# cyberfabric/cyberfabric-core

Hardware: AMD Instinct MI355X
Metric: tokens/sec + p50 TTFT via llm-gateway REST /v1/chat/completions (higher is better)
Workload: dtype bf16; 1 GPU; model=llama3-8b, global_batch=2048, seq_len=512, parallelism=dp1(worker fleet)

## Files before the change

### csrc/attn_paged.hip

```cpp
#include <float.h>

#include "common.h"

#define ATTN_BS 16

template <int GROUP, int D>
__global__ __launch_bounds__(256) void paged_attn_kernel(
    bf16* __restrict__ out, const bf16* __restrict__ q,
    const bf16* __restrict__ k_cache, const bf16* __restrict__ v_cache,
    const int* __restrict__ block_tables, const int* __restrict__ ctx_lens,
    const int* __restrict__ row_seq, int max_blocks, int num_kv_heads,
    float scale, long q_stride) {
  constexpr int SLICE = D / 4;
  constexpr int VPL = D / 64;
  constexpr bool QREG = (GROUP <= 4);
  const int row = blockIdx.x;
  const int kvh = blockIdx.y;
  const int H = num_kv_heads * GROUP;
  const int ctx = ctx_lens[row];
  const int table = row_seq ? row_seq[row] : row;
  const int* bt = block_tables + (long)table * max_blocks;
  const int nblocks = (ctx + ATTN_BS - 1) / ATTN_BS;

  __shared__ __attribute__((aligned(16))) float q_lds[GROUP][D];
// ... 149 lines not shown
  }
  __syncthreads();
  for (int i = threadIdx.x; i < GROUP * D; i += 256) {
    const int h = i / D, d = i % D;
    float M = fmaxf(fmaxf(comb_m[0][h], comb_m[1][h]),
                    fmaxf(comb_m[2][h], comb_m[3][h]));
    float o = 0.f, L = 0.f;
    #pragma unroll
    for (int w = 0; w < 4; ++w) {
      const float f = (comb_m[w][h] == -FLT_MAX) ? 0.f
                                                 : __expf(comb_m[w][h] - M);
      o += f * comb_o[w][h][d];
      L += f * comb_l[w][h];
    }
    *(unsigned short*)(out + ((long)row * H + kvh * GROUP + h) * D + d) =
        f2bf(o / L);
  }
}


DEV float dot2_bf16(unsigned a, unsigned b, float c) {
  asm("v_dot2_f32_bf16 %0, %1, %2, %0" : "+v"(c) : "v"(a), "v"(b));
  return c;
}

typedef __attribute__((ext_vector_type(2))) float float2v;

DEV unsigned pk_bf16(float a, float b) {
  unsigned r;
  asm("v_cvt_pk_bf16_f32 %0, %1, %2" : "=v"(r) : "v"(a), "v"(b));
  return r;
}

template <int GROUP, bool KV8>
__global__ __launch_bounds__(256) void paged_attn_v3_kernel(
    bf16* __restrict__ out, const bf16* __restrict__ q,
    const bf16* __restrict__ k_cache, const bf16* __restrict__ v_cache,
    const int* __restrict__ block_tables, const int* __restrict__ ctx_lens,
    const int* __restrict__ row_seq, int max_blocks, int num_kv_heads,
    float scale, long q_stride, int h_total, int g_stride, int h_off,
    float* __restrict__ partial) {
  constexpr int D = 128;
  const int row = blockIdx.x;
  const int kvh = blockIdx.y;
  const int split = gridDim.z;
  const int H = h_total;
  const int ctx = ctx_lens[row];
  const int table = row_seq ? row_seq[row] : row;
  const int* bt = block_tables + (long)table * max_blocks;
  const int nblocks = (ctx + ATTN_BS - 1) / ATTN_BS;

  __shared__ __attribute__((aligned(16))) float sc[4][GROUP][ATTN_BS];
  __shared__ __attribute__((aligned(16))) float comb_o[4][GROUP][D];
  __shared__ float comb_m[4][GROUP];
  __shared__ float comb_l[4][GROUP];

  const int wid = threadIdx.x >> 6;
  const int lane = threadIdx.x & 63;
  const int t_loc = lane >> 3;
  const int sl = lane & 7;
  const int ds = lane & 15;
  const int g = lane >> 4;

  unsigned q_pk[GROUP][8];
  {
    const bf16* qp = q + (long)row * q_stride
                     + ((long)kvh * g_stride + h_off) * D + sl * 16;
    #pragma unroll
    for (int h = 0; h < GROUP; ++h) {
      uint4 a = *reinterpret_cast<const uint4*>(qp + h * D);
      uint4 b = *reinterpret_cast<const uint4*>(qp + h * D + 8);
      q_pk[h][0] = a.x; q_pk[h][1] = a.y; q_pk[h][2] = a.z; q_pk[h][3] = a.w;
      q_pk[h][4] = b.x; q_pk[h][5] = b.y; q_pk[h][6] = b.z; q_pk[h][7] = b.w;
    }
  }

  float m[GROUP], l[GROUP];
  float2 acc[GROUP][4];
  #pragma unroll
  for (int h = 0; h < GROUP; ++h) {
    m[h] = -FLT_MAX; l[h] = 0.f;
    #pragma unroll
    for (int j = 0; j < 4; ++j) acc[h][j] = make_float2(0.f, 0.f);
  }

  for (int b = 4 * blockIdx.z + wid; b < nblocks; b += 4 * split) {
    const long blk = bt[b];
    const int nb = min(ATTN_BS, ctx - b * ATTN_BS);
    const long page_off = ((blk * num_kv_heads + kvh) * ATTN_BS) * D;
    const bf16* pbase = k_cache + page_off;
    const bf16* vbase = v_cache + page_off;
    const unsigned char* pbase8 =
        reinterpret_cast<const unsigned char*>(k_cache) + page_off;
    const unsigned char* vbase8 =
        reinterpret_cast<const unsigned char*>(v_cache) + page_off;
    uint4 kr[2][KV8 ? 1 : 2];
    uint4 vr4[KV8 ? 1 : 4];
    uint2 vr2[KV8 ? 4 : 1];
    #pragma unroll
    for (int p = 0; p < 2; ++p) {
      if constexpr (KV8) {
        kr[p][0] = *reinterpret_cast<const uint4*>(
            pbase8 + (p * 8 + t_loc) * D + sl * 16);
      } else {
        const bf16* kp = pbase + (p * 8 + t_loc) * D + sl * 16;
        kr[p][0] = *reinterpret_cast<const uint4*>(kp);
        kr[p][1] = *reinterpret_cast<const uint4*>(kp + 8);
      }
    }
    #pragma unroll
    for (int i = 0; i < 4; ++i) {
      if constexpr (KV8)
        vr2[i] = *reinterpret_cast<const uint2*>(vbase8 + (4 * g + i) * D
                                                 + ds * 8);
      else
        vr4[i] = *reinterpret_cast<const uint4*>(vbase + (4 * g + i) * D
                                                 + ds * 8);
    }
    float s[GROUP][2];
    #pragma unroll
    for (int p = 0; p < 2; ++p) {
      unsigned kw[8];
      if constexpr (KV8) {
        const unsigned* kq = reinterpret_cast<const unsigned*>(&kr[p][0]);
        #pragma unroll
        for (int i = 0; i < 4; ++i) {
          float2v lo = __builtin_amdgcn_cvt_pk_f32_fp8(kq[i], false);
          float2v hi = __builtin_amdgcn_cvt_pk_f32_fp8(kq[i], true);
          kw[2 * i] = pk_bf16(lo.x, lo.y);
          kw[2 * i + 1] = pk_bf16(hi.x, hi.y);
        }
      } else {
        #pragma unroll
        for (int j = 0; j < 8; ++j)
          kw[j] = reinterpret_cast<const unsigned*>(&kr[p][0])[j];
      }
      #pragma unroll
      for (int h = 0; h < GROUP; ++h) {
        float d = 0.f;
        #pragma unroll
        for (int j = 0; j < 8; ++j) d = dot2_bf16(q_pk[h][j], kw[j], d);
        d += __shfl_xor(d, 1);
        d += __shfl_xor(d, 2);
        d += __shfl_xor(d, 4);
        const int tok = p * 8 + t_loc;
        s[h][p] = (tok < nb) ? d * scale : -FLT_MAX;
      }
    }
    #pragma unroll
    for (int h = 0; h < GROUP; ++h) {
      float bm = fmaxf(s[h][0], s[h][1]);
// ... 24 lines not shown
    #pragma unroll
    for (int h = 0; h < GROUP; ++h)
      p4[h] = *reinterpret_cast<const float4*>(&sc[wid][h][4 * g]);
    #pragma unroll
    for (int i = 0; i < 4; ++i) {
      float2 vf[4];
      if constexpr (KV8) {
        const unsigned* vw = reinterpret_cast<const unsigned*>(&vr2[i]);
        #pragma unroll
        for (int jj = 0; jj < 2; ++jj) {
          float2v lo = __builtin_amdgcn_cvt_pk_f32_fp8(vw[jj], false);
          float2v hi = __builtin_amdgcn_cvt_pk_f32_fp8(vw[jj], true);
          vf[2 * jj].x = lo.x; vf[2 * jj].y = lo.y;
          vf[2 * jj + 1].x = hi.x; vf[2 * jj + 1].y = hi.y;
        }
      } else {
        const unsigned* vw = reinterpret_cast<const unsigned*>(&vr4[i]);
        #pragma unroll
        for (int j = 0; j < 4; ++j) {
          vf[j].x = bf2f((unsigned short)(vw[j] & 0xffff));
          vf[j].y = bf2f((unsigned short)(vw[j] >> 16));
        }
      }
      #pragma unroll
      for (int h = 0; h < GROUP; ++h) {
        const float p = (&p4[h].x)[i];
        #pragma unroll
        for (int j = 0; j < 4; ++j) {
          acc[h][j].x += p * vf[j].x;
          acc[h][j].y += p * vf[j].y;
        }
      }
    }
  }

  #pragma unroll
  for (int h = 0; h < GROUP; ++h) {
    #pragma unroll
    for (int j = 0; j < 4; ++j) {
      acc[h][j].x += __shfl_xor(acc[h][j].x, 16);
      acc[h][j].x += __shfl_xor(acc[h][j].x, 32);
      acc[h][j].y += __shfl_xor(acc[h][j].y, 16);
      acc[h][j].y += __shfl_xor(acc[h][j].y, 32);
    }
  }
  if (lane < 16) {
    #pragma unroll
    for (int h = 0; h < GROUP; ++h)
      #pragma unroll
      for (int j = 0; j < 4; ++j)
        *reinterpret_cast<float2*>(&comb_o[wid][h][ds * 8 + j * 2]) =
            acc[h][j];
  }
  if (lane == 0) {
    #pragma unroll
    for (int h = 0; h < GROUP; ++h) {
      comb_m[wid][h] = m[h];
      comb_l[wid][h] = l[h];
    }
  }
  __syncthreads();
  for (int i = threadIdx.x; i < GROUP * D; i += 256) {
    const int h = i / D, d = i % D;
    float M = fmaxf(fmaxf(comb_m[0][h], comb_m[1][h]),
                    fmaxf(comb_m[2][h], comb_m[3][h]));
    float o = 0.f, L = 0.f;
// ... 37 lines not shown
      const float* pz = base + (long)z * GROUP * (D + 2);
      const float mz = pz[D];
      const float f = (mz == -FLT_MAX) ? 0.f : __expf(mz - M);
      o += f * pz[d];
      L += f * pz[D + 1];
    }
    *(unsigned short*)(out +
        ((long)row * h_total + kvh * g_stride + h + h_off) * D + d) =
        f2bf(o / L);
  }
}

void launch_paged_attn(bf16* out, const bf16* q, const bf16* k_cache,
                       const bf16* v_cache, const int* block_tables,
                       const int* ctx_lens, const int* row_seq,
                       long num_rows, int num_kv_heads, int group, int D,
                       int max_blocks, int block_size, float scale,
                       long q_stride, float* split_ws, int split,
                       bool kv_fp8, hipStream_t stream) {
  if (block_size != ATTN_BS)
    throw std::runtime_error("paged_attn: block_size must be 16");
  if (D == 128 && (group <= 4 || group == 8)) {
    const int calls = (group == 8) ? 2 : 1;
    const int g = (group == 8) ? 4 : group;
    const int h_total = num_kv_heads * group;
    for (int c = 0; c < calls; ++c) {
      const int h_off = c * 4;
      dim3 grid((unsigned)num_rows, (unsigned)num_kv_heads,
                (unsigned)split);
      dim3 mgrid((unsigned)num_rows, (unsigned)num_kv_heads);
      #define CASE3(G)                                                      \
        if (g == G) {                                                       \
          if (kv_fp8)                                                       \
            paged_attn_v3_kernel<G, true><<<grid, 256, 0, stream>>>(        \
                out, q, k_cache, v_cache, block_tables, ctx_lens, row_seq,  \
                max_blocks, num_kv_heads, scale, q_stride, h_total, group,  \
                h_off, split_ws);                                           \
          else                                                              \
            paged_attn_v3_kernel<G, false><<<grid, 256, 0, stream>>>(       \
                out, q, k_cache, v_cache, block_tables, ctx_lens, row_seq,  \
                max_blocks, num_kv_heads, scale, q_stride, h_total, group,  \
                h_off, split_ws);                                           \
          if (split > 1)                                                    \
            paged_attn_v3_merge_kernel<G><<<mgrid, 256, 0, stream>>>(       \
                out, split_ws, split, h_total, group, h_off);               \
        }
      CASE3(1) CASE3(2) CASE3(4)
      #undef CASE3
    }
    return;
  }
  if (split != 1)
    throw std::runtime_error("paged_attn: split needs the v3 path");
  if (kv_fp8)
    throw std::runtime_error("paged_attn: fp8 KV needs head_dim 128");
  dim3 grid((unsigned)num_rows, (unsigned)num_kv_heads);
  #define CASE(G, DD)                                                       \
    if (group == G && D == DD) {                                            \
      paged_attn_kernel<G, DD><<<grid, 256, 0, stream>>>(                   \
          out, q, k_cache, v_cache, block_tables, ctx_lens, row_seq,        \
          max_blocks, num_kv_heads, scale, q_stride);                       \
      return;                                                               \
    }
  CASE(1, 64) CASE(2, 64) CASE(4, 64) CASE(8, 64)
  #undef CASE
  throw std::runtime_error("paged_attn: unsupported (group, head_dim)");
}
```

### csrc/bindings.cpp

```cpp
#include <torch/extension.h>

#include <c10/hip/HIPStream.h>
#include <hip/hip_bf16.h>

#include <stdexcept>

using bf16 = __hip_bfloat16;

void launch_rmsnorm(bf16*, const bf16*, const bf16*, float, long, int,
                    hipStream_t);
void launch_fused_add_rmsnorm(bf16*, bf16*, const bf16*, float, long, int,
                              hipStream_t);
void launch_rope_kv_append(bf16*, bf16*, const bf16*, const long*,
                           const float*, const long*, bf16*, bf16*, long,
                           int, int, int, int, long, long, long, bool,
                           hipStream_t);
void launch_paged_attn(bf16*, const bf16*, const bf16*, const bf16*,
                       const int*, const int*, const int*, long, int, int,
                       int, int, int, float, long, float*, int, bool,
                       hipStream_t);
void launch_attn_prefill_mfma(bf16*, const bf16*, const bf16*,
                              const bf16*, const int*, int, int, int, int,
                              int, float, long, long, long, hipStream_t);
void launch_attn_prefill_paged_mfma(bf16*, const bf16*, const bf16*,
                                    const bf16*, const int*, const int*,
                                    const int*, int, int, int, int, int, int,
                                    int, float, long, bool, hipStream_t);
void launch_silu_mul(bf16*, const bf16*, long, int, hipStream_t);
void launch_quant_fp8(unsigned char*, float*, const bf16*, long, int, long,
                      hipStream_t);
void launch_fused_add_rmsnorm_fp8(unsigned char*, float*, const bf16*,
                                  bf16*, const bf16*, float, long, int,
                                  hipStream_t);
void launch_silu_mul_fp8(unsigned char*, float*, const bf16*, long, int,
                         hipStream_t);
void launch_moe_align(int*, int*, int*, const int*, int, int, int,
                      hipStream_t);
void launch_moe_gemm(bf16*, float*, const bf16*, const bf16*, const int*,
                     const int*, int, int, int, int, int, hipStream_t);
void launch_moe_combine(bf16*, const bf16*, const float*, const int*, long,
                        int, int, hipStream_t);
void launch_moe_gemm_fp8(bf16*, float*, const unsigned char*, const float*,
                         const unsigned char*, const float*, const int*,
                         const int*, int, int, int, int, int, hipStream_t);
void launch_greedy_sample(long*, const bf16*, long, int, hipStream_t);
void launch_inv_cdf_sample(long*, const float*, const float*, long, int,
                           hipStream_t);
void launch_decode_advance(long*, long*, int*, long*, int*, const long*,
                           const int*, int, int, int, hipStream_t);

namespace {

hipStream_t stream() {
// ... 68 lines not shown
                torch::Tensor ctx_lens,
                c10::optional<torch::Tensor> row_seq, double scale,
                c10::optional<torch::Tensor> split_ws, long split) {
  check(out, torch::kBFloat16, "out");
  check_qkv_view(q, "q");
  check(block_tables, torch::kInt32, "block_tables");
  check(ctx_lens, torch::kInt32, "ctx_lens");
  const long R = q.size(0);
  const int H = (int)q.size(1), D = (int)q.size(2);
  const int KV = (int)k_cache.size(1), BS = (int)k_cache.size(2);
  TORCH_CHECK(H % KV == 0, "GQA group");
  const int* rs = nullptr;
  if (row_seq.has_value()) {
    check(*row_seq, torch::kInt32, "row_seq");
    rs = row_seq->data_ptr<int>();
  }
  float* ws = nullptr;
  if (split > 1) {
    TORCH_CHECK(split_ws.has_value(), "split>1 needs a workspace");
    check(*split_ws, torch::kFloat, "split_ws");
    TORCH_CHECK(split_ws->numel() >= R * KV * split * (H / KV) * (D + 2),
                "split_ws too small");
    ws = split_ws->data_ptr<float>();
  }
  const bool kv_fp8 =
      k_cache.scalar_type() == torch::kFloat8_e4m3fn;
  TORCH_CHECK(v_cache.scalar_type() == k_cache.scalar_type(),
              "k/v cache dtype mismatch");
  launch_paged_attn(bf(out), cbf(q), cbf(k_cache), cbf(v_cache),
                    block_tables.data_ptr<int>(), ctx_lens.data_ptr<int>(),
                    rs, R, KV, H / KV, D, (int)block_tables.size(1), BS,
                    (float)scale, q.stride(0), ws, (int)split, kv_fp8,
                    stream());
}

void attn_prefill_mfma(torch::Tensor out, torch::Tensor q, torch::Tensor k,
                       torch::Tensor v, torch::Tensor seq_start,
                       long max_seqlen, double scale) {
  check(out, torch::kBFloat16, "out");
  check_qkv_view(q, "q");
  check_qkv_view(k, "k");
  check_qkv_view(v, "v");
  check(seq_start, torch::kInt32, "seq_start");
  const int H = (int)q.size(1), D = (int)q.size(2);
  const int KV = (int)k.size(1);
  launch_attn_prefill_mfma(
      bf(out), cbf(q), cbf(k), cbf(v), seq_start.data_ptr<int>(),
      (int)seq_start.numel() - 1, (int)max_seqlen, H, KV, D, (float)scale,
      q.stride(0), k.stride(0), v.stride(0), stream());
}

void attn_prefill_paged_mfma(torch::Tensor out, torch::Tensor q,
                             torch::Tensor k_cache, torch::Tensor v_cache,
                             torch::Tensor block_tables,
                             torch::Tensor seq_start,
                             torch::Tensor ctx_start, long max_seqlen,
                             double scale) {
  check(out, torch::kBFloat16, "out");
  check_qkv_view(q, "q");
  TORCH_CHECK(out.dim() == 3 && out.sizes() == q.sizes(),
              "out must be [T, H, D] like q");
  TORCH_CHECK(q.size(2) == 128,
              "attn_prefill_paged_mfma: head_dim must be 128, got ",
              q.size(2));
  TORCH_CHECK(k_cache.is_cuda() && v_cache.is_cuda() &&
                  k_cache.is_contiguous() && v_cache.is_contiguous(),
// ... 193 lines not shown
  check(sorted_ids, torch::kInt, "sorted_ids");
  check(tile_expert, torch::kInt, "tile_expert");
  TORCH_CHECK(wq.dim() == 3, "wq must be [E, N, K]");
  float* skp = nullptr;
  if (splitk > 1) {
    TORCH_CHECK(skw.has_value(),
                "moe_gemm_fp8: splitk>1 needs a workspace");
    check(*skw, torch::kFloat, "skw");
    TORCH_CHECK(skw->numel() >= splitk * out.numel(),
                "moe_gemm_fp8: workspace too small");
    skp = skw->data_ptr<float>();
  }
  launch_moe_gemm_fp8(bf(out), skp, u8(xq), xs.data_ptr<float>(), u8(wq),
                      ws.data_ptr<float>(), sorted_ids.data_ptr<int>(),
                      tile_expert.data_ptr<int>(),
                      (int)tile_expert.numel(), (int)wq.size(1),
                      (int)wq.size(2), (int)gather_div, (int)splitk,
                      stream());
}

PYBIND11_MODULE(TORCH_EXTENSION_NAME, m) {
  m.doc() = "HyperSpot-AMD gfx950 (CDNA4) kernels";
  m.def("rmsnorm", &rmsnorm);
  m.def("quant_fp8", &quant_fp8);
  m.def("fused_add_rmsnorm_fp8", &fused_add_rmsnorm_fp8);
  m.def("silu_mul_fp8", &silu_mul_fp8);
  m.def("moe_align", &moe_align);
  m.def("moe_gemm", &moe_gemm);
  m.def("moe_combine", &moe_combine);
  m.def("moe_gemm_fp8", &moe_gemm_fp8);
  m.def("fused_add_rmsnorm", &fused_add_rmsnorm);
  m.def("rope_kv_append", &rope_kv_append);
  m.def("paged_attn", &paged_attn);
  m.def("attn_prefill_mfma", &attn_prefill_mfma);
  m.def("attn_prefill_paged_mfma", &attn_prefill_paged_mfma);
  m.def("silu_mul", &silu_mul);
  m.def("greedy_sample", &greedy_sample);
  m.def("inv_cdf_sample", &inv_cdf_sample);
  m.def("decode_advance", &decode_advance);
}
```

### csrc/common.h

```cpp
#pragma once

#include <hip/hip_runtime.h>
#include <hip/hip_bf16.h>

#define WAVE 64
#define DEV __device__ __forceinline__

using bf16 = __hip_bfloat16;

DEV float bf2f(unsigned short u) {
  union { unsigned int i; float f; } c;
  c.i = (unsigned int)u << 16;
  return c.f;
}

DEV unsigned short f2bf(float f) {
  union { float f; unsigned int i; } c;
  c.f = f;
  unsigned int lsb = (c.i >> 16) & 1;
  c.i += 0x7fffu + lsb;
  return (unsigned short)(c.i >> 16);
}

struct bf16x8 { uint4 raw; };

DEV bf16x8 load_bf16x8(const bf16* p) {
  bf16x8 r;
  r.raw = *reinterpret_cast<const uint4*>(p);
  return r;
}

DEV void store_bf16x8(bf16* p, const bf16x8& v) {
  *reinterpret_cast<uint4*>(p) = v.raw;
}

DEV float bf16x8_get(const bf16x8& v, int i) {
  unsigned int w = (&v.raw.x)[i >> 1];
  return bf2f((unsigned short)(i & 1 ? w >> 16 : w & 0xffff));
}

DEV void bf16x8_set(bf16x8& v, int i, float f) {
  unsigned int* w = &(&v.raw.x)[i >> 1];
  unsigned short b = f2bf(f);
  if (i & 1) *w = (*w & 0x0000ffffu) | ((unsigned int)b << 16);
  else       *w = (*w & 0xffff0000u) | b;
}

DEV float wave_reduce_sum(float v) {
  #pragma unroll
  for (int o = 32; o > 0; o >>= 1) v += __shfl_xor(v, o);
  return v;
}

DEV float wave_reduce_max(float v) {
// ... 34 lines not shown
```

### csrc/rope_kv.hip

```cpp
#include "common.h"

template <int D, bool KV8>
__global__ __launch_bounds__(256) void rope_kv_append_kernel(
    bf16* __restrict__ q, bf16* __restrict__ k, const bf16* __restrict__ v,
    const long* __restrict__ positions, const float* __restrict__ cos_sin,
    const long* __restrict__ slot_mapping, bf16* __restrict__ k_cache,
    bf16* __restrict__ v_cache, int H, int KV, int block_size,
    long qs_stride, long ks_stride, long vs_stride) {
  constexpr int HALF = D / 2;
  __shared__ float cs[D];
  const long t = blockIdx.x;
  const long pos = positions[t];
  const long slot = slot_mapping[t];
  const long blk = slot >= 0 ? slot / block_size : 0;
  const long off = slot >= 0 ? slot % block_size : 0;

  for (int i = threadIdx.x; i < D; i += 256)
    cs[i] = cos_sin[pos * D + i];
  __syncthreads();

  const int PAIR2 = HALF / 2;
  const int total_q = H * PAIR2;
  for (int u = threadIdx.x; u < total_q; u += 256) {
    const int h = u / PAIR2, j = (u % PAIR2) * 2;
    bf16* base = q + t * qs_stride + h * D;
    ushort2 lo = *reinterpret_cast<ushort2*>(base + j);
    ushort2 hi = *reinterpret_cast<ushort2*>(base + HALF + j);
    float c0 = cs[j], c1 = cs[j + 1];
    float s0 = cs[HALF + j], s1 = cs[HALF + j + 1];
    float x0 = bf2f(lo.x), x1 = bf2f(lo.y);
    float y0 = bf2f(hi.x), y1 = bf2f(hi.y);
    lo.x = f2bf(x0 * c0 - y0 * s0); lo.y = f2bf(x1 * c1 - y1 * s1);
    hi.x = f2bf(y0 * c0 + x0 * s0); hi.y = f2bf(y1 * c1 + x1 * s1);
    *reinterpret_cast<ushort2*>(base + j) = lo;
    *reinterpret_cast<ushort2*>(base + HALF + j) = hi;
  }
  const int total_k = KV * PAIR2;
  for (int u = threadIdx.x; u < total_k; u += 256) {
    const int h = u / PAIR2, j = (u % PAIR2) * 2;
    bf16* base = k + t * ks_stride + h * D;
    ushort2 lo = *reinterpret_cast<ushort2*>(base + j);
    ushort2 hi = *reinterpret_cast<ushort2*>(base + HALF + j);
    float c0 = cs[j], c1 = cs[j + 1];
    float s0 = cs[HALF + j], s1 = cs[HALF + j + 1];
    float x0 = bf2f(lo.x), x1 = bf2f(lo.y);
    float y0 = bf2f(hi.x), y1 = bf2f(hi.y);
    const float r0 = x0 * c0 - y0 * s0, r1 = x1 * c1 - y1 * s1;
    const float r2 = y0 * c0 + x0 * s0, r3 = y1 * c1 + x1 * s1;
    lo.x = f2bf(r0); lo.y = f2bf(r1);
    hi.x = f2bf(r2); hi.y = f2bf(r3);
    *reinterpret_cast<ushort2*>(base + j) = lo;
    *reinterpret_cast<ushort2*>(base + HALF + j) = hi;
    if (slot >= 0) {
      if constexpr (KV8) {
        unsigned char* kc = reinterpret_cast<unsigned char*>(k_cache) +
            (((blk * KV + h) * block_size + off) * D);
        unsigned plo = __builtin_amdgcn_cvt_pk_fp8_f32(r0, r1, 0u, false);
        unsigned phi = __builtin_amdgcn_cvt_pk_fp8_f32(r2, r3, 0u, false);
        *reinterpret_cast<unsigned short*>(kc + j) = (unsigned short)plo;
        *reinterpret_cast<unsigned short*>(kc + HALF + j) =
            (unsigned short)phi;
      } else {
        bf16* kc = k_cache + (((blk * KV + h) * block_size + off) * D);
        *reinterpret_cast<ushort2*>(kc + j) = lo;
        *reinterpret_cast<ushort2*>(kc + HALF + j) = hi;
      }
    }
  }
  if (slot >= 0) {
    const int total_v = KV * D / 8;
    for (int u = threadIdx.x; u < total_v; u += 256) {
      const int h = u / (D / 8), j = (u % (D / 8)) * 8;
      const bf16* src = v + t * vs_stride + h * D + j;
      if constexpr (KV8) {
        bf16x8 vv = load_bf16x8(src);
        unsigned w0 = 0, w1 = 0;
        w0 = __builtin_amdgcn_cvt_pk_fp8_f32(bf16x8_get(vv, 0),
                                             bf16x8_get(vv, 1), w0, false);
        w0 = __builtin_amdgcn_cvt_pk_fp8_f32(bf16x8_get(vv, 2),
                                             bf16x8_get(vv, 3), w0, true);
        w1 = __builtin_amdgcn_cvt_pk_fp8_f32(bf16x8_get(vv, 4),
// ... 38 lines not shown
```

### hyperspot/models/llama.py

```python

from __future__ import annotations

from dataclasses import dataclass
from typing import List, Optional

import torch
from torch import nn

from hyperspot import ops
from hyperspot.engine.config import ModelSpec
from hyperspot.ops.torch_ref import rope_cos_sin
from hyperspot.parallel import (QKVParallelLinear, RowParallelLinear,
                                MergedColumnParallelLinear)
from hyperspot.parallel.state import get_tp_size


@dataclass
class ForwardMeta:

    mode: str
    positions: torch.Tensor
    slot_mapping: torch.Tensor
    seq_start: Optional[torch.Tensor] = None
    max_seqlen: int = 0
    row_seq: Optional[torch.Tensor] = None
    ctx_lens: Optional[torch.Tensor] = None
    block_tables: Optional[torch.Tensor] = None
    seq_lens: Optional[torch.Tensor] = None
    logits_indices: Optional[torch.Tensor] = None
    return_hidden: bool = False
    fresh_prefill: bool = True
    ctx_start: Optional[torch.Tensor] = None
    paged_mfma: bool = False


class Attention(nn.Module):
    def __init__(self, spec: ModelSpec, layer_idx: int, dtype: torch.dtype):
        super().__init__()
        self.layer_idx = layer_idx
        self.head_dim = spec.head_dim
        self.scale = spec.head_dim ** -0.5
        self.qkv = QKVParallelLinear(spec.hidden_size, spec.head_dim,
                                     spec.num_heads, spec.num_kv_heads, dtype,
                                     seed_tag=layer_idx * 10 + 1)
        self.o_proj = RowParallelLinear(
            spec.num_heads * spec.head_dim, spec.hidden_size, dtype,
            seed_tag=layer_idx * 10 + 4)

    def forward(self, x, meta: ForwardMeta,
                kv_cache: torch.Tensor, cos_sin: torch.Tensor) -> torch.Tensor:
        q, k, v = self.qkv(x)
        T = q.shape[0]
        k_cache, v_cache = kv_cache[0], kv_cache[1]
        ops.rope_kv_append(q, k, v, meta.positions, cos_sin,
                           meta.slot_mapping, k_cache, v_cache)
        o = ops.attention(q, k, v, k_cache, v_cache, meta, self.scale)
        o = o.view(T, -1)
        if self.o_proj.quant == "fp8" and o.is_cuda:
            o = ops.quant_fp8(o)
        return self.o_proj(o)


class LlamaMLP(nn.Module):
    def __init__(self, spec: ModelSpec, layer_idx: int, dtype: torch.dtype):
        super().__init__()
        self.gate_up = MergedColumnParallelLinear(
            spec.hidden_size, [spec.intermediate_size, spec.intermediate_size],
            dtype, seed_tag=layer_idx * 10 + 5)
        self.down = RowParallelLinear(spec.intermediate_size,
                                      spec.hidden_size, dtype,
                                      seed_tag=layer_idx * 10 + 7)
        self.tp = get_tp_size()
        self.inter_shard = spec.intermediate_size // self.tp

    def forward(self, x) -> torch.Tensor:
        gu = self.gate_up(x)
        if self.down.quant == "fp8" and gu.is_cuda:
            return self.down(ops.silu_mul_q(gu))
        return self.down(ops.silu_mul(gu))


class DecoderLayer(nn.Module):
    def __init__(self, spec: ModelSpec, layer_idx: int, dtype: torch.dtype,
                 mlp_cls=LlamaMLP):
        super().__init__()
        self.input_norm_w = nn.Parameter(
            torch.ones(spec.hidden_size, dtype=dtype), requires_grad=False)
        self.post_norm_w = nn.Parameter(
            torch.ones(spec.hidden_size, dtype=dtype), requires_grad=False)
# ... 70 lines not shown
```

### hyperspot/ops/__init__.py

```python

from __future__ import annotations

from typing import NamedTuple

import torch

from . import torch_ref

_C = None
_C_ERR: Exception | None = None
try:
    from hyperspot import _C as _C
except Exception as e:
    _C_ERR = e


def have_native() -> bool:
    return _C is not None


def _native():
    if _C is None:
        raise RuntimeError(
            "hyperspot._C (gfx950 HIP extension) is not built but a GPU tensor "
# ... 70 lines not shown

_PAGED_MFMA_MAX_PER_ROW = 16


def attention(q: torch.Tensor, k: torch.Tensor, v: torch.Tensor,
              k_cache: torch.Tensor, v_cache: torch.Tensor, meta,
              scale: float) -> torch.Tensor:
    if meta.mode == "decode":
        return paged_attn_decode(q, k_cache, v_cache, meta.block_tables,
                                 meta.seq_lens, scale)
    if q.is_cuda:
        out = torch.empty(q.shape, dtype=q.dtype, device=q.device)
        if q.shape[-1] == 128 and getattr(meta, "fresh_prefill", True):
            _native().attn_prefill_mfma(out, q, k, v, meta.seq_start,
                                        meta.max_seqlen, scale)
        elif q.shape[-1] == 128 and getattr(meta, "paged_mfma", False) \
                and meta.max_seqlen > _PAGED_MFMA_MAX_PER_ROW:
            if meta.ctx_start is None:
                raise RuntimeError(
                    "prefill over the paged cache needs meta.ctx_start")
            _native().attn_prefill_paged_mfma(
                out, q, k_cache, v_cache, meta.block_tables, meta.seq_start,
                meta.ctx_start, meta.max_seqlen, scale)
        else:
            _native().paged_attn(out, q, k_cache, v_cache,
                                 meta.block_tables, meta.ctx_lens,
                                 meta.row_seq, scale, None, 1)
        return out
    if getattr(meta, "fresh_prefill", True):
        return torch_ref.prefill_attn(q, k, v, meta.seq_start, scale)
    return torch_ref.prefill_attn_paged(q, k_cache, v_cache,
                                        meta.block_tables, meta.ctx_lens,
                                        meta.row_seq, scale)


def silu_mul(gate_up: torch.Tensor) -> torch.Tensor:
    if gate_up.is_cuda:
        i = gate_up.shape[-1] // 2
        out = torch.empty(*gate_up.shape[:-1], i, dtype=gate_up.dtype,
                          device=gate_up.device)
        _native().silu_mul(out, gate_up)
        return out
    return torch_ref.silu_mul(gate_up)


class QTensor(NamedTuple):

    data: torch.Tensor
    scale: torch.Tensor


def quant_fp8(x: torch.Tensor) -> QTensor:
    assert x.is_cuda
    T, K = x.shape
    out = torch.empty(T, K, dtype=torch.float8_e4m3fn, device=x.device)
    scales = torch.empty(T, dtype=torch.float32, device=x.device)
    _native().quant_fp8(out, scales, x)
    return QTensor(out, scales)


def fused_add_rmsnorm_q(x: torch.Tensor, residual: torch.Tensor,
                        weight: torch.Tensor, eps: float):
    assert x.is_cuda
    T, K = x.shape
    out = torch.empty(T, K, dtype=torch.float8_e4m3fn, device=x.device)
    scales = torch.empty(T, dtype=torch.float32, device=x.device)
# ... 152 lines not shown
```

Before: 40290 tokens/s.

## Fuse decode RoPE and KV-cache append into the paged attention kernel

Adds a FUSED variant of the v3 paged decode attention kernel. It applies RoPE to q and to the new k in registers, writes the new k/v token into the paged cache from the wave that owns the last page, and then runs attention, so the separate rope_kv_append launch and its q round trip through memory go away. The change also prefetches the next block-table entry, clamps loads in partial pages, and enables the fused path by default through an environment flag. The price is extra shuffles and register pressure, plus an in-kernel ordering dependency between the cache write and the read of the last page, which is handled with wavefront fences.

Result: no change. 40000 tokens/s (-0.7%).

```diff
diff --git a/csrc/attn_paged.hip b/csrc/attn_paged.hip
--- a/csrc/attn_paged.hip
+++ b/csrc/attn_paged.hip
@@ -205,14 +205,57 @@
   return r;
 }
 
-template <int GROUP, bool KV8>
+struct FusedRope {
+  const bf16* k_new;
+  const bf16* v_new;
+  const long* positions;
+  const float* cos_sin;
+  const long* slot_mapping;
+  long k_stride, v_stride;
+};
+
+template <bool FUSED> struct kv_pool_ptr {
+  typedef const bf16* __restrict__ type;
+};
+template <> struct kv_pool_ptr<true> { typedef bf16* type; };
+
+DEV void pack16_bf16(const float* r, uint4& a, uint4& b) {
+  unsigned w[8];
+  #pragma unroll
+  for (int i = 0; i < 8; ++i)
+    w[i] = (unsigned)f2bf(r[2 * i]) | ((unsigned)f2bf(r[2 * i + 1]) << 16);
+  a = make_uint4(w[0], w[1], w[2], w[3]);
+  b = make_uint4(w[4], w[5], w[6], w[7]);
+}
+
+DEV void rope_slice16(const unsigned* own, const float* c, const float* s,
+                      bool lo_half, float* r) {
+  #pragma unroll
+  for (int i = 0; i < 8; ++i) {
+    const unsigned oth = __shfl_xor(own[i], 4);
+    const unsigned xw = lo_half ? own[i] : oth;
+    const unsigned yw = lo_half ? oth : own[i];
+    float l0, h0, l1, h1;
+    rope_rotate(bf2f((unsigned short)(xw & 0xffff)),
+                bf2f((unsigned short)(yw & 0xffff)), c[2 * i], s[2 * i],
+                l0, h0);
+    rope_rotate(bf2f((unsigned short)(xw >> 16)),
+                bf2f((unsigned short)(yw >> 16)), c[2 * i + 1],
+                s[2 * i + 1], l1, h1);
+    r[2 * i] = lo_half ? l0 : h0;
+    r[2 * i + 1] = lo_half ? l1 : h1;
+  }
+}
+
+template <int GROUP, bool KV8, bool FUSED>
 __global__ __launch_bounds__(256) void paged_attn_v3_kernel(
     bf16* __restrict__ out, const bf16* __restrict__ q,
-    const bf16* __restrict__ k_cache, const bf16* __restrict__ v_cache,
+    typename kv_pool_ptr<FUSED>::type k_cache,
+    typename kv_pool_ptr<FUSED>::type v_cache,
     const int* __restrict__ block_tables, const int* __restrict__ ctx_lens,
     const int* __restrict__ row_seq, int max_blocks, int num_kv_heads,
     float scale, long q_stride, int h_total, int g_stride, int h_off,
-    float* __restrict__ partial) {
+    float* __restrict__ partial, FusedRope fz) {
   constexpr int D = 128;
   const int row = blockIdx.x;
   const int kvh = blockIdx.y;
@@ -228,26 +271,13 @@
   __shared__ float comb_m[4][GROUP];
   __shared__ float comb_l[4][GROUP];
 
-  const int wid = threadIdx.x >> 6;
+  const int wid = __builtin_amdgcn_readfirstlane(threadIdx.x >> 6);
   const int lane = threadIdx.x & 63;
   const int t_loc = lane >> 3;
   const int sl = lane & 7;
   const int ds = lane & 15;
   const int g = lane >> 4;
 
-  unsigned q_pk[GROUP][8];
-  {
-    const bf16* qp = q + (long)row * q_stride
-                     + ((long)kvh * g_stride + h_off) * D + sl * 16;
-    #pragma unroll
-    for (int h = 0; h < GROUP; ++h) {
-      uint4 a = *reinterpret_cast<const uint4*>(qp + h * D);
-      uint4 b = *reinterpret_cast<const uint4*>(qp + h * D + 8);
-      q_pk[h][0] = a.x; q_pk[h][1] = a.y; q_pk[h][2] = a.z; q_pk[h][3] = a.w;
-      q_pk[h][4] = b.x; q_pk[h][5] = b.y; q_pk[h][6] = b.z; q_pk[h][7] = b.w;
-    }
-  }
-
   float m[GROUP], l[GROUP];
   float2 acc[GROUP][4];
   #pragma unroll
@@ -257,8 +287,13 @@
     for (int j = 0; j < 4; ++j) acc[h][j] = make_float2(0.f, 0.f);
   }
 
-  for (int b = 4 * blockIdx.z + wid; b < nblocks; b += 4 * split) {
-    const long blk = bt[b];
+  unsigned q_pk[GROUP][8];
+  uint4 kr[2][KV8 ? 1 : 2];
+  uint4 vr4[KV8 ? 1 : 4];
+  uint2 vr2[KV8 ? 4 : 1];
+
+  auto load_page = [&](int b, int blk_id) {
+    const long blk = blk_id;
     const int nb = min(ATTN_BS, ctx - b * ATTN_BS);
     const long page_off = ((blk * num_kv_heads + kvh) * ATTN_BS) * D;
     const bf16* pbase = k_cache + page_off;
@@ -267,29 +302,38 @@
         reinterpret_cast<const unsigned char*>(k_cache) + page_off;
     const unsigned char* vbase8 =
         reinterpret_cast<const unsigned char*>(v_cache) + page_off;
-    uint4 kr[2][KV8 ? 1 : 2];
-    uint4 vr4[KV8 ? 1 : 4];
-    uint2 vr2[KV8 ? 4 : 1];
-    #pragma unroll
-    for (int p = 0; p < 2; ++p) {
-      if constexpr (KV8) {
-        kr[p][0] = *reinterpret_cast<const uint4*>(
-            pbase8 + (p * 8 + t_loc) * D + sl * 16);
-      } else {
-        const bf16* kp = pbase + (p * 8 + t_loc) * D + sl * 16;
-        kr[p][0] = *reinterpret_cast<const uint4*>(kp);
-        kr[p][1] = *reinterpret_cast<const uint4*>(kp + 8);
-      }
-    }
-    #pragma unroll
-    for (int i = 0; i < 4; ++i) {
-      if constexpr (KV8)
-        vr2[i] = *reinterpret_cast<const uint2*>(vbase8 + (4 * g + i) * D
-                                                 + ds * 8);
-      else
-        vr4[i] = *reinterpret_cast<const uint4*>(vbase + (4 * g + i) * D
-                                                 + ds * 8);
-    }
+    auto load_rows = [&](auto clamp) {
+      #pragma unroll
+      for (int p = 0; p < 2; ++p) {
+        const int t = clamp(p * 8 + t_loc);
+        if constexpr (KV8) {
+          kr[p][0] = *reinterpret_cast<const uint4*>(pbase8 + t * D
+                                                     + sl * 16);
+        } else {
+          const bf16* kp = pbase + t * D + sl * 16;
+          kr[p][0] = *reinterpret_cast<const uint4*>(kp);
+          kr[p][1] = *reinterpret_cast<const uint4*>(kp + 8);
+        }
+      }
+      #pragma unroll
+      for (int i = 0; i < 4; ++i) {
+        const int t = clamp(4 * g + i);
+        if constexpr (KV8)
+          vr2[i] = *reinterpret_cast<const uint2*>(vbase8 + t * D + ds * 8);
+        else
+          vr4[i] = *reinterpret_cast<const uint4*>(vbase + t * D + ds * 8);
+      }
+    };
+    if (nb == ATTN_BS) {
+      load_rows([](int t) { return t; });
+    } else {
+      load_rows([nb](int t) { return min(t, nb - 1); });
+      asm volatile("" ::: "memory");
+    }
+  };
+
+  auto compute_page = [&](int b) {
+    const int nb = min(ATTN_BS, ctx - b * ATTN_BS);
     float s[GROUP][2];
     #pragma unroll
     for (int p = 0; p < 2; ++p) {
@@ -380,6 +424,135 @@
         }
       }
     }
+  };
+
+  int b = 4 * blockIdx.z + wid;
+  int blk = (b < nblocks) ? bt[b] : 0;
+  if constexpr (!FUSED) {
+    const bf16* qp = q + (long)row * q_stride
+                     + ((long)kvh * g_stride + h_off) * D + sl * 16;
+    #pragma unroll
+    for (int h = 0; h < GROUP; ++h) {
+      const uint4 a = *reinterpret_cast<const uint4*>(qp + h * D);
+      const uint4 c = *reinterpret_cast<const uint4*>(qp + h * D + 8);
+      q_pk[h][0] = a.x; q_pk[h][1] = a.y; q_pk[h][2] = a.z; q_pk[h][3] = a.w;
+      q_pk[h][4] = c.x; q_pk[h][5] = c.y; q_pk[h][6] = c.z; q_pk[h][7] = c.w;
+    }
+  } else {
+    const long pos = fz.positions[row];
+    const long slot = fz.slot_mapping[row];
+    const bool lo_half = sl < 4;
+    const int hs = (sl & 3) * 16;
+    const int last = nblocks - 1;
+    const bool owner = slot >= 0 && ((last & 3) == wid);
+    const int h_mine = t_loc & (GROUP - 1);
+    unsigned qr[8];
+    float cs_c[16], cs_s[16];
+    {
+      const bf16* qp = q + (long)row * q_stride
+                       + ((long)kvh * g_stride + h_off + h_mine) * D + sl * 16;
+      const uint4 a = *reinterpret_cast<const uint4*>(qp);
+      const uint4 c = *reinterpret_cast<const uint4*>(qp + 8);
+      qr[0] = a.x; qr[1] = a.y; qr[2] = a.z; qr[3] = a.w;
+      qr[4] = c.x; qr[5] = c.y; qr[6] = c.z; qr[7] = c.w;
+      const float* cp = fz.cos_sin + pos * D + hs;
+      #pragma unroll
+      for (int i = 0; i < 4; ++i) {
+        const float4 c4 = *reinterpret_cast<const float4*>(cp + 4 * i);
+        const float4 s4 = *reinterpret_cast<const float4*>(cp + 64 + 4 * i);
+        cs_c[4 * i] = c4.x; cs_c[4 * i + 1] = c4.y;
+        cs_c[4 * i + 2] = c4.z; cs_c[4 * i + 3] = c4.w;
+        cs_s[4 * i] = s4.x; cs_s[4 * i + 1] = s4.y;
+        cs_s[4 * i + 2] = s4.z; cs_s[4 * i + 3] = s4.w;
+      }
+    }
+    unsigned kn[8];
+    uint4 vn = make_uint4(0u, 0u, 0u, 0u);
+    #pragma unroll
+    for (int i = 0; i < 8; ++i) kn[i] = 0u;
+    if (owner) {
+      const bf16* kp = fz.k_new + (long)row * fz.k_stride + (long)kvh * D
+                       + sl * 16;
+      const uint4 a = *reinterpret_cast<const uint4*>(kp);
+      const uint4 c = *reinterpret_cast<const uint4*>(kp + 8);
+      kn[0] = a.x; kn[1] = a.y; kn[2] = a.z; kn[3] = a.w;
+      kn[4] = c.x; kn[5] = c.y; kn[6] = c.z; kn[7] = c.w;
+      if (g == 0)
+        vn = *reinterpret_cast<const uint4*>(
+            fz.v_new + (long)row * fz.v_stride + (long)kvh * D + ds * 8);
+    }
+
+    auto append = [&]() {
+      const long slot_off =
+          (((slot >> 4) * num_kv_heads + kvh) * ATTN_BS + (slot & 15)) * D;
+      float r[16];
+      rope_slice16(kn, cs_c, cs_s, lo_half, r);
+      if (t_loc == 0) {
+        if constexpr (KV8) {
+          unsigned w[4];
+          #pragma unroll
+          for (int i = 0; i < 4; ++i) {
+            w[i] = __builtin_amdgcn_cvt_pk_fp8_f32(r[4 * i], r[4 * i + 1],
+                                                   0u, false);
+            w[i] = __builtin_amdgcn_cvt_pk_fp8_f32(r[4 * i + 2],
+                                                   r[4 * i + 3], w[i], true);
+          }
+          *reinterpret_cast<uint4*>(reinterpret_cast<unsigned char*>(k_cache)
+                                    + slot_off + sl * 16) =
+              make_uint4(w[0], w[1], w[2], w[3]);
+        } else {
+          uint4 a, c;
+          pack16_bf16(r, a, c);
+          bf16* kc = k_cache + slot_off + sl * 16;
+          *reinterpret_cast<uint4*>(kc) = a;
+          *reinterpret_cast<uint4*>(kc + 8) = c;
+        }
+      }
+      if (g == 0) {
+        if constexpr (KV8) {
+          bf16x8 vv; vv.raw = vn;
+          unsigned w0 = 0, w1 = 0;
+          w0 = __builtin_amdgcn_cvt_pk_fp8_f32(bf16x8_get(vv, 0),
+                                               bf16x8_get(vv, 1), w0, false);
+          w0 = __builtin_amdgcn_cvt_pk_fp8_f32(bf16x8_get(vv, 2),
+                                               bf16x8_get(vv, 3), w0, true);
+          w1 = __builtin_amdgcn_cvt_pk_fp8_f32(bf16x8_get(vv, 4),
+                                               bf16x8_get(vv, 5), w1, false);
+          w1 = __builtin_amdgcn_cvt_pk_fp8_f32(bf16x8_get(vv, 6),
+                                               bf16x8_get(vv, 7), w1, true);
+          *reinterpret_cast<uint2*>(reinterpret_cast<unsigned char*>(v_cache)
+                                    + slot_off + ds * 8) = make_uint2(w0, w1);
+        } else {
+          *reinterpret_cast<uint4*>(v_cache + slot_off + ds * 8) = vn;
+        }
+      }
+    };
+    {
+      float r[16];
+      rope_slice16(qr, cs_c, cs_s, lo_half, r);
+      uint4 a, c;
+      pack16_bf16(r, a, c);
+      const unsigned mine[8] = {a.x, a.y, a.z, a.w, c.x, c.y, c.z, c.w};
+      #pragma unroll
+      for (int h = 0; h < GROUP; ++h)
+        #pragma unroll
+        for (int j = 0; j < 8; ++j)
+          q_pk[h][j] = __shfl(mine[j], h * 8 + sl);
+    }
+    if (owner) append();
+  }
+  for (; b < nblocks; b += 4 * split) {
+    const int nxt = (b + 4 * split < nblocks) ? bt[b + 4 * split] : 0;
+    if constexpr (FUSED) {
+      if (b == nblocks - 1) {
+        __builtin_amdgcn_fence(__ATOMIC_RELEASE, "wavefront");
+        __builtin_amdgcn_s_waitcnt(0x0f70);
+        __builtin_amdgcn_fence(__ATOMIC_ACQUIRE, "wavefront");
+      }
+    }
+    load_page(b, blk);
+    compute_page(b);
+    blk = nxt;
   }
 
   #pragma unroll
@@ -483,15 +656,15 @@
       #define CASE3(G)                                                      \
         if (g == G) {                                                       \
           if (kv_fp8)                                                       \
-            paged_attn_v3_kernel<G, true><<<grid, 256, 0, stream>>>(        \
+            paged_attn_v3_kernel<G, true, false><<<grid, 256, 0, stream>>>( \
                 out, q, k_cache, v_cache, block_tables, ctx_lens, row_seq,  \
                 max_blocks, num_kv_heads, scale, q_stride, h_total, group,  \
-                h_off, split_ws);                                           \
+                h_off, split_ws, FusedRope{});                              \
           else                                                              \
-            paged_attn_v3_kernel<G, false><<<grid, 256, 0, stream>>>(       \
+            paged_attn_v3_kernel<G, false, false><<<grid, 256, 0, stream>>>(\
                 out, q, k_cache, v_cache, block_tables, ctx_lens, row_seq,  \
                 max_blocks, num_kv_heads, scale, q_stride, h_total, group,  \
-                h_off, split_ws);                                           \
+                h_off, split_ws, FusedRope{});                              \
           if (split > 1)                                                    \
             paged_attn_v3_merge_kernel<G><<<mgrid, 256, 0, stream>>>(       \
                 out, split_ws, split, h_total, group, h_off);               \
@@ -517,3 +690,39 @@
   #undef CASE
   throw std::runtime_error("paged_attn: unsupported (group, head_dim)");
 }
+
+void launch_paged_attn_fused(bf16* out, const bf16* q, const bf16* k_new,
+                             const bf16* v_new, const long* positions,
+                             const float* cos_sin, const long* slot_mapping,
+                             bf16* k_cache, bf16* v_cache,
+                             const int* block_tables, const int* ctx_lens,
+                             long num_rows, int num_kv_heads, int group,
+                             int D, int max_blocks, int block_size,
+                             float scale, long q_stride, long k_stride,
+                             long v_stride, bool kv_fp8,
+                             hipStream_t stream) {
+  if (block_size != ATTN_BS)
+    throw std::runtime_error("paged_attn_fused: block_size must be 16");
+  if (D != 128 || (group != 1 && group != 2 && group != 4))
+    throw std::runtime_error(
+        "paged_attn_fused: needs head_dim 128 and GROUP in {1, 2, 4}");
+  const FusedRope fz{k_new, v_new, positions, cos_sin, slot_mapping,
+                     k_stride, v_stride};
+  dim3 grid((unsigned)num_rows, (unsigned)num_kv_heads, 1u);
+  const int h_total = num_kv_heads * group;
+  #define CASEF(G)                                                          \
+    if (group == G) {                                                       \
+      if (kv_fp8)                                                           \
+        paged_attn_v3_kernel<G, true, true><<<grid, 256, 0, stream>>>(      \
+            out, q, k_cache, v_cache, block_tables, ctx_lens, nullptr,      \
+            max_blocks, num_kv_heads, scale, q_stride, h_total, group, 0,   \
+            nullptr, fz);                                                   \
+      else                                                                  \
+        paged_attn_v3_kernel<G, false, true><<<grid, 256, 0, stream>>>(     \
+            out, q, k_cache, v_cache, block_tables, ctx_lens, nullptr,      \
+            max_blocks, num_kv_heads, scale, q_stride, h_total, group, 0,   \
+            nullptr, fz);                                                   \
+    }
+  CASEF(1) CASEF(2) CASEF(4)
+  #undef CASEF
+}
diff --git a/csrc/bindings.cpp b/csrc/bindings.cpp
--- a/csrc/bindings.cpp
+++ b/csrc/bindings.cpp
@@ -19,6 +19,11 @@
                        const int*, const int*, const int*, long, int, int,
                        int, int, int, float, long, float*, int, bool,
                        hipStream_t);
+void launch_paged_attn_fused(bf16*, const bf16*, const bf16*, const bf16*,
+                             const long*, const float*, const long*, bf16*,
+                             bf16*, const int*, const int*, long, int, int,
+                             int, int, int, float, long, long, long, bool,
+                             hipStream_t);
 void launch_attn_prefill_mfma(bf16*, const bf16*, const bf16*,
                               const bf16*, const int*, int, int, int, int,
                               int, float, long, long, long, hipStream_t);
@@ -153,6 +158,59 @@
                     rs, R, KV, H / KV, D, (int)block_tables.size(1), BS,
                     (float)scale, q.stride(0), ws, (int)split, kv_fp8,
                     stream());
+}
+
+void paged_attn_fused(torch::Tensor out, torch::Tensor q, torch::Tensor k,
+                      torch::Tensor v, torch::Tensor positions,
+                      torch::Tensor cos_sin, torch::Tensor slot_mapping,
+                      torch::Tensor k_cache, torch::Tensor v_cache,
+                      torch::Tensor block_tables, torch::Tensor ctx_lens,
+                      double scale) {
+  check(out, torch::kBFloat16, "out");
+  check_qkv_view(q, "q");
+  check_qkv_view(k, "k");
+  check_qkv_view(v, "v");
+  check(cos_sin, torch::kFloat32, "cos_sin");
+  check(positions, torch::kInt64, "positions");
+  check(slot_mapping, torch::kInt64, "slot_mapping");
+  check(block_tables, torch::kInt32, "block_tables");
+  check(ctx_lens, torch::kInt32, "ctx_lens");
+  const long R = q.size(0);
+  const int H = (int)q.size(1), D = (int)q.size(2);
+  TORCH_CHECK(k_cache.is_cuda() && v_cache.is_cuda() &&
+                  k_cache.is_contiguous() && v_cache.is_contiguous() &&
+                  k_cache.dim() == 4 && k_cache.sizes() == v_cache.sizes(),
+              "k_cache/v_cache must be contiguous [NB, KV, 16, D] on GPU");
+  const int KV = (int)k_cache.size(1), BS = (int)k_cache.size(2);
+  TORCH_CHECK(out.numel() == q.numel(), "out must be [T, H, D] like q");
+  TORCH_CHECK(D == 128 && k_cache.size(3) == D, "head_dim must be 128");
+  TORCH_CHECK(KV > 0 && H % KV == 0 && H / KV <= 4 && H / KV != 3,
+              "GQA group must be 1, 2 or 4");
+  TORCH_CHECK(k.size(0) == R && v.size(0) == R && k.size(1) == KV &&
+                  v.size(1) == KV && k.size(2) == D && v.size(2) == D,
+              "k/v must be [T, KV, D]");
+  TORCH_CHECK(q.stride(0) % 8 == 0 && k.stride(0) % 8 == 0 &&
+                  v.stride(0) % 8 == 0 && q.storage_offset() % 8 == 0 &&
+                  k.storage_offset() % 8 == 0 && v.storage_offset() % 8 == 0,
+              "q/k/v rows must be 16-byte aligned");
+  TORCH_CHECK(positions.numel() == R && slot_mapping.numel() == R &&
+                  ctx_lens.numel() == R,
+              "positions/slot_mapping/ctx_lens must have one entry per row");
+  TORCH_CHECK(block_tables.dim() == 2 && block_tables.size(0) == R,
+              "block_tables must be [T, max_blocks]");
+  TORCH_CHECK(cos_sin.dim() == 2 && cos_sin.size(1) == D,
+              "cos_sin must be [max_pos, D]");
+  const bool kv_fp8 = k_cache.scalar_type() == torch::kFloat8_e4m3fn;
+  TORCH_CHECK(kv_fp8 || k_cache.scalar_type() == torch::kBFloat16,
+              "cache dtype must be bfloat16 or float8_e4m3fn");
+  TORCH_CHECK(v_cache.scalar_type() == k_cache.scalar_type(),
+              "k/v cache dtype mismatch");
+  launch_paged_attn_fused(
+      bf(out), cbf(q), cbf(k), cbf(v), positions.data_ptr<long>(),
+      cos_sin.data_ptr<float>(), slot_mapping.data_ptr<long>(), bf(k_cache),
+      bf(v_cache), block_tables.data_ptr<int>(), ctx_lens.data_ptr<int>(), R,
+      KV, H / KV, D, (int)block_tables.size(1), BS, (float)scale,
+      q.stride(0), k.stride(0), v.stride(0), kv_fp8, stream());
 }
 
 void attn_prefill_mfma(torch::Tensor out, torch::Tensor q, torch::Tensor k,
@@ -412,6 +470,7 @@
   m.def("fused_add_rmsnorm", &fused_add_rmsnorm);
   m.def("rope_kv_append", &rope_kv_append);
   m.def("paged_attn", &paged_attn);
+  m.def("paged_attn_fused", &paged_attn_fused);
   m.def("attn_prefill_mfma", &attn_prefill_mfma);
   m.def("attn_prefill_paged_mfma", &attn_prefill_paged_mfma);
   m.def("silu_mul", &silu_mul);
diff --git a/csrc/common.h b/csrc/common.h
--- a/csrc/common.h
+++ b/csrc/common.h
@@ -20,6 +20,15 @@
   unsigned int lsb = (c.i >> 16) & 1;
   c.i += 0x7fffu + lsb;
   return (unsigned short)(c.i >> 16);
+}
+
+DEV void rope_rotate(float x, float y, float c, float s, float& lo,
+                     float& hi) {
+  #pragma clang fp contract(off)
+  const float ys = y * s;
+  const float xs = x * s;
+  lo = __builtin_fmaf(x, c, -ys);
+  hi = __builtin_fmaf(y, c, xs);
 }
 
 struct bf16x8 { uint4 raw; };
diff --git a/csrc/rope_kv.hip b/csrc/rope_kv.hip
--- a/csrc/rope_kv.hip
+++ b/csrc/rope_kv.hip
@@ -30,8 +30,11 @@
     float s0 = cs[HALF + j], s1 = cs[HALF + j + 1];
     float x0 = bf2f(lo.x), x1 = bf2f(lo.y);
     float y0 = bf2f(hi.x), y1 = bf2f(hi.y);
-    lo.x = f2bf(x0 * c0 - y0 * s0); lo.y = f2bf(x1 * c1 - y1 * s1);
-    hi.x = f2bf(y0 * c0 + x0 * s0); hi.y = f2bf(y1 * c1 + x1 * s1);
+    float r0, r1, r2, r3;
+    rope_rotate(x0, y0, c0, s0, r0, r2);
+    rope_rotate(x1, y1, c1, s1, r1, r3);
+    lo.x = f2bf(r0); lo.y = f2bf(r1);
+    hi.x = f2bf(r2); hi.y = f2bf(r3);
     *reinterpret_cast<ushort2*>(base + j) = lo;
     *reinterpret_cast<ushort2*>(base + HALF + j) = hi;
   }
@@ -45,8 +48,9 @@
     float s0 = cs[HALF + j], s1 = cs[HALF + j + 1];
     float x0 = bf2f(lo.x), x1 = bf2f(lo.y);
     float y0 = bf2f(hi.x), y1 = bf2f(hi.y);
-    const float r0 = x0 * c0 - y0 * s0, r1 = x1 * c1 - y1 * s1;
-    const float r2 = y0 * c0 + x0 * s0, r3 = y1 * c1 + x1 * s1;
+    float r0, r1, r2, r3;
+    rope_rotate(x0, y0, c0, s0, r0, r2);
+    rope_rotate(x1, y1, c1, s1, r1, r3);
     lo.x = f2bf(r0); lo.y = f2bf(r1);
     hi.x = f2bf(r2); hi.y = f2bf(r3);
     *reinterpret_cast<ushort2*>(base + j) = lo;
diff --git a/hyperspot/models/llama.py b/hyperspot/models/llama.py
--- a/hyperspot/models/llama.py
+++ b/hyperspot/models/llama.py
@@ -52,9 +52,9 @@
         q, k, v = self.qkv(x)
         T = q.shape[0]
         k_cache, v_cache = kv_cache[0], kv_cache[1]
-        ops.rope_kv_append(q, k, v, meta.positions, cos_sin,
-                           meta.slot_mapping, k_cache, v_cache)
-        o = ops.attention(q, k, v, k_cache, v_cache, meta, self.scale)
+        o = ops.rope_attention(q, k, v, meta.positions, cos_sin,
+                               meta.slot_mapping, k_cache, v_cache, meta,
+                               self.scale)
         o = o.view(T, -1)
         if self.o_proj.quant == "fp8" and o.is_cuda:
             o = ops.quant_fp8(o)
diff --git a/hyperspot/ops/__init__.py b/hyperspot/ops/__init__.py
--- a/hyperspot/ops/__init__.py
+++ b/hyperspot/ops/__init__.py
@@ -126,6 +126,34 @@
     return torch_ref.prefill_attn_paged(q, k_cache, v_cache,
                                         meta.block_tables, meta.ctx_lens,
                                         meta.row_seq, scale)
+
+
+_FUSED_DECODE_ROPE = os.environ.get("HYPERSPOT_FUSED_DECODE_ROPE", "1") != "0"
+
+
+def fused_decode_rope_applies(mode: str, head_dim: int, group: int, rows: int,
+                              kvh: int, kv_dtype: torch.dtype) -> bool:
+    return (_FUSED_DECODE_ROPE and mode == "decode" and head_dim == 128
+            and group in (1, 2, 4) and _attn_split(rows, kvh) == 1
+            and kv_dtype in (torch.bfloat16, torch.float8_e4m3fn))
+
+
+def rope_attention(q: torch.Tensor, k: torch.Tensor, v: torch.Tensor,
+                   positions: torch.Tensor, cos_sin: torch.Tensor,
+                   slot_mapping: torch.Tensor, k_cache: torch.Tensor,
+                   v_cache: torch.Tensor, meta, scale: float) -> torch.Tensor:
+    kvh = k_cache.shape[1]
+    if q.is_cuda and fused_decode_rope_applies(
+            meta.mode, q.shape[-1], q.shape[1] // kvh, q.shape[0], kvh,
+            k_cache.dtype):
+        out = torch.empty(q.shape, dtype=q.dtype, device=q.device)
+        _native().paged_attn_fused(out, q, k, v, positions, cos_sin,
+                                   slot_mapping, k_cache, v_cache,
+                                   meta.block_tables, meta.seq_lens, scale)
+        return out
+    rope_kv_append(q, k, v, positions, cos_sin, slot_mapping, k_cache,
+                   v_cache)
+    return attention(q, k, v, k_cache, v_cache, meta, scale)
 
 
 def silu_mul(gate_up: torch.Tensor) -> torch.Tensor:
```
